# WLBF/flex-gpu-scheduler

Hardware: AMD Instinct MI355X
Metric: pods/sec sched throughput + p99 PodGroup gang-admit latency, 1/2/4/8-GPU groups (higher is better)
Workload: dtype int64

## Files before the change

csrc/api/types.cc:

```cpp
#include "api/types.h"

#include <algorithm>
#include <charconv>
#include <chrono>
#include <cstdio>
#include <cstdlib>
#include <limits>
#include <mutex>
#include <unordered_set>

#include "api/storage.h"

namespace xsched {

namespace {
int64_t days_from_civil(int64_t y, unsigned m, unsigned d) {
  y -= m <= 2;
  const int64_t era = (y >= 0 ? y : y - 399) / 400;
  const unsigned yoe = static_cast<unsigned>(y - era * 400);
  const unsigned doy = (153 * (m + (m > 2 ? -3 : 9)) + 2) / 5 + d - 1;
  const unsigned doe = yoe * 365 + yoe / 4 - yoe / 100 + doy;
  return era * 146097 + static_cast<int64_t>(doe) - 719468;
}
void civil_from_days(int64_t z, int64_t* y, unsigned* m, unsigned* d) {
// ... 342 lines not shown
    gpu.kind = GpuAssignment::Kind::Partition;
  } else if (limits.has(mid)) {
    gpu.kind = GpuAssignment::Kind::Memory;
    gpu.memory = limits.get(mid);
  } else {
    return;
  }
  gpu.gpus = std::move(gpus);
  gpu.partitions = std::move(parts);
}

const std::string& IStr::intern(std::string_view v) {
  static const std::string* kCommon[] = {new std::string(kDefaultSchedulerName), new std::string("PreemptLowerPriority"),
                                         new std::string("")};
  for (const std::string* c : kCommon)
    if (*c == v) return *c;
  static std::mutex mu;
  static auto* table = new std::unordered_set<std::string>();
  std::lock_guard<std::mutex> g(mu);
  return *table->emplace(v).first;
}

uint64_t pg_key_of(std::string_view full) {
  uint64_t h = 1469598103934665603ULL;
  for (unsigned char c : full) {
    h ^= c;
    h *= 1099511628211ULL;
  }
  return h ? h : 1;
}

std::shared_ptr<Pod> Pod::from_json(const Json& obj, const GpuNames& gn) {
  auto p = std::make_shared<Pod>();
  p->meta = ObjectMeta::from_json(obj);
  const Json& spec = obj["spec"];
  const Json& status = obj["status"];
  p->spec_hash = json_hash(spec, 1469598103934665603ULL, "nodeName");
  if (spec["nodeName"].as_string().empty()) {
    const Json& md = obj["metadata"];
    uint64_t h = json_hash(md["namespace"], p->spec_hash);
    p->template_hash = json_hash(md["annotations"], h);
  }
  if (spec["schedulerName"].is_string()) p->scheduler_name = spec["schedulerName"].as_string();
  p->node_name = spec["nodeName"].as_string();
  p->priority_class_name = spec["priorityClassName"].as_string();
  p->priority = as_i32(spec["priority"]);
  if (spec["preemptionPolicy"].is_string()) p->preemption_policy = spec["preemptionPolicy"].as_string();
  {
    std::vector<Container> cs, ics;
    for (const auto& c : spec["containers"].items()) cs.push_back(parse_container(c));
    for (const auto& c : spec["initContainers"].items()) ics.push_back(parse_container(c));
    p->containers = std::move(cs);
    p->init_containers = std::move(ics);
  }
  p->volumes = parse_pod_volumes(spec, p->meta.name);
  auto res = std::make_shared<PodRes>();
  res->overhead = Res::from_json(spec["overhead"]);
  p->node_selector = strmap_from_json(spec["nodeSelector"]);
  if (const Json* na = spec.path({"affinity", "nodeAffinity"})) {
    if (const Json* req = na->get("requiredDuringSchedulingIgnoredDuringExecution")) {
      p->has_required_node_affinity = true;
      for (const auto& t : (*req)["nodeSelectorTerms"].items()) p->required_node_terms.push_back(parse_term(t));
    }
    for (const auto& t : (*na)["preferredDuringSchedulingIgnoredDuringExecution"].items()) {
      PreferredSchedulingTerm pt;
      pt.weight = as_i32(t["weight"]);
      pt.pref = parse_term(t["preference"]);
      p->preferred_node_terms.push_back(std::move(pt));
    }
  }
  if (const Json* pa = spec.path({"affinity", "podAffinity"}))
    parse_pod_affinity(*pa, &p->pod_affinity_required, &p->pod_affinity_preferred);
  if (const Json* paa = spec.path({"affinity", "podAntiAffinity"}))
    parse_pod_affinity(*paa, &p->pod_anti_affinity_required, &p->pod_anti_affinity_preferred);
  for (const auto& c : spec["topologySpreadConstraints"].items()) {
    TopologySpreadConstraint tc;
    tc.max_skew = as_i32(c["maxSkew"], 1);
    tc.topology_key = c["topologyKey"].as_string();
    tc.hard = c["whenUnsatisfiable"].str_or("DoNotSchedule") != "ScheduleAnyway";
    tc.selector = LabelSelector::from_json(c.get("labelSelector"));
    p->spread_constraints.push_back(std::move(tc));
  }
  for (const auto& t : spec["tolerations"].items()) {
    Toleration tol;
    tol.key = t["key"].as_string();
    tol.op = t["operator"].str_or("Equal");
    tol.value = t["value"].as_string();
    tol.effect = t["effect"].as_string();
    if (t["tolerationSeconds"].is_number()) tol.toleration_seconds = t["tolerationSeconds"].as_int();
    p->tolerations.push_back(std::move(tol));
  }
  if (status["phase"].is_string()) p->phase = status["phase"].as_string();
  p->nominated_node_name = status["nominatedNodeName"].as_string();
  if (status["startTime"].is_string()) p->start_time = parse_rfc3339(status["startTime"].as_string());
  for (const auto& c : status["conditions"].items())
    if (c["type"].as_string() == "PodScheduled" && c["status"].as_string() == "True")
      p->scheduled_at = parse_rfc3339(c["lastTransitionTime"].as_string());

  Res sum;
  for (const auto& c : p->containers) {
    add_saturating(sum, c.requests);
    add_saturating(res->limit_sum, c.limits);
    Res nz;
    nz.set(kCPU, c.requests.has(kCPU) && c.requests.get(kCPU) != 0 ? c.requests.get(kCPU) : kDefaultMilliCPU);
    nz.set(kMemory, c.requests.has(kMemory) && c.requests.get(kMemory) != 0 ? c.requests.get(kMemory) : kDefaultMemory);
    add_saturating(res->nonzero_request, nz);
    for (const auto& port : c.ports)
      if (port.host_port > 0) p->host_ports.push_back(port);
  }
  if (p->containers.empty()) {
    res->nonzero_request.set(kCPU, 0);
    res->nonzero_request.set(kMemory, 0);
  }
  for (const auto& c : p->init_containers) {
    sum.set_max(c.requests);
    Res nz;
    nz.set(kCPU, c.requests.has(kCPU) && c.requests.get(kCPU) != 0 ? c.requests.get(kCPU) : kDefaultMilliCPU);
    nz.set(kMemory, c.requests.has(kMemory) && c.requests.get(kMemory) != 0 ? c.requests.get(kMemory) : kDefaultMemory);
    res->nonzero_request.set_max(nz);
  }
  add_saturating(sum, res->overhead);
  add_saturating(res->nonzero_request, res->overhead);
  res->request = sum;
  p->res = std::move(res);
  p->qos = compute_qos(*p);
  if (const std::string* pg = p->meta.label(kPodGroupLabel)) {
    p->pod_group = *pg;
    p->pg_key = pg_key_of(p->pg_full_name());
  }
  p->gpu_demand = compute_gpu_demand(*p, gn);
  p->recompute_gpu_assignment(gn);
  return p;
}

int partitions_for_mode(const std::string& mode) {
  std::string m;
  for (char c : mode) m.push_back(static_cast<char>(std::tolower(static_cast<unsigned char>(c))));
  if (m == "spx") return 1;
  if (m == "dpx") return 2;
  if (m == "qpx") return 4;
  if (m == "cpx") return 8;
  return 0;
}

bool node_selector_term_matches(const NodeSelectorTerm& t, const Node& n) {
  if (t.match_expressions.empty() && t.match_fields.empty()) return false;
  for (const auto& r : t.match_expressions)
    if (!match_requirement(r, n.meta.labels)) return false;
  for (const auto& r : t.match_fields) {
    if (r.key != "metadata.name") return false;
    StrMap f{{"metadata.name", n.name()}};
    if (!match_requirement(r, f)) return false;
  }
  return true;
}

bool pod_matches_node_selector_and_affinity(const Pod& p, const Node& n) {
  for (const auto& kv : p.node_selector) {
    const std::string* v = n.meta.label(kv.first);
    if (!v || *v != kv.second) return false;
  }
  if (!p.has_required_node_affinity) return true;
  for (const auto& t : p.required_node_terms)
    if (node_selector_term_matches(t, n)) return true;
  return false;
// ... 228 lines not shown
```

csrc/api/types.h:

```cpp
#pragma once

#include <atomic>
#include <cstdint>
#include <memory>
#include <optional>
#include <string>
#include <string_view>
#include <unordered_map>
#include <vector>

#include "api/resource.h"
#include "common/json.h"

namespace xsched {

inline constexpr const char* kPodGroupLabel = "pod-group.scheduling.sigs.k8s.io";
inline constexpr const char* kDefaultSchedulerName = "default-scheduler";

using MicroTime = int64_t;
MicroTime parse_rfc3339(const std::string& s);
std::string format_rfc3339(MicroTime t);
MicroTime wall_now_us();

using StrMap = std::vector<std::pair<std::string, std::string>>;
// ... 239 lines not shown
  };
  mutable ListedMark listed;
  struct HeapTag {
    uint8_t v = 0;
    HeapTag() = default;
    HeapTag(const HeapTag&) {}
    HeapTag& operator=(const HeapTag&) { return *this; }
  };
  mutable HeapTag heap_tag;

  std::shared_ptr<const PodRes> res = PodRes::empty();
  const Res& request() const { return res->request; }
  const Res& nonzero_request() const { return res->nonzero_request; }
  const Res& limit_sum() const { return res->limit_sum; }
  const Res& overhead() const { return res->overhead; }
  QoS qos = QoS::BestEffort;
  std::string pod_group;
  uint64_t pg_key = 0;
  std::shared_ptr<Gang> gang;
  std::vector<ContainerPort> host_ports;
  GpuAssignment gpu;
  GpuDemand gpu_demand;
  uint64_t template_hash = 0;
  uint64_t spec_hash = 0;

  const std::string& ns() const { return meta.ns; }
  const std::string& name() const { return meta.name; }
  const std::string& uid() const { return meta.uid; }
  std::string key() const { return meta.ns + "/" + meta.name; }
  bool terminating() const { return meta.deletion != 0; }
  std::string pg_full_name() const { return pod_group.empty() ? std::string() : meta.ns + "/" + pod_group; }

  static std::shared_ptr<Pod> from_json(const Json& obj, const GpuNames& gn = default_gpu_names());
  void recompute_gpu_assignment(const GpuNames& gn = default_gpu_names());
  void set_gpu_assignment(std::vector<int> gpus, std::vector<std::pair<int, int>> parts,
                          const GpuNames& gn = default_gpu_names());
};
using PodPtr = std::shared_ptr<Pod>;

uint64_t pg_key_of(std::string_view full_name);

struct Node {
  ObjectMeta meta;
  Res allocatable, capacity;
  bool unschedulable = false;
  std::vector<Taint> taints;
  std::vector<ContainerImage> images;
  std::unordered_map<std::string, int64_t> image_sizes;
  bool has_prefer_no_schedule = false;
  bool foreign_hostname = false;
  int gpu_count = 0;
  std::vector<int> gpu_partitions;
  std::vector<int> gpu_numa;
  std::vector<uint8_t> gpu_xcd_faults;
  int64_t gpu_memory_per_gpu = 0;
  const std::string& name() const { return meta.name; }
  static std::shared_ptr<Node> from_json(const Json& obj, const GpuNames& gn = default_gpu_names());
};
using NodePtr = std::shared_ptr<Node>;

bool node_selector_term_matches(const NodeSelectorTerm& t, const Node& n);
bool pod_matches_node_selector_and_affinity(const Pod& p, const Node& n);

struct PodGroup {
  ObjectMeta meta;
  int32_t min_member = 0;
// ... 96 lines not shown
```

csrc/python/bindings.cc:

```cpp
#include <pybind11/functional.h>
#include <pybind11/pybind11.h>
#include <pybind11/stl.h>

#include <atomic>
#include <map>
#include <set>

#include "api/types.h"
#include "common/alloc.h"
#include "common/json.h"
#include "common/quantity.h"
#include "rest/kube.h"
#include "scheduler/openloop.h"
#include "common/log.h"
#include "apiserver/apiserver.h"
#include "scheduler/scheduler.h"
#include "store/store.h"
#include "telemetry/amdsmi_sampler.h"
#include "tools/sampler.h"

namespace py = pybind11;
using namespace xsched;

namespace {
// ... 82 lines not shown
};

py::dict pod_struct_summary(const Pod& pod);

py::dict pod_summary(const Json& obj) { return pod_struct_summary(*Pod::from_json(obj)); }

py::dict pod_struct_summary(const Pod& pod) {
  const Pod* p = &pod;
  py::dict d;
  d["key"] = p->key();
  d["request"] = to_py(p->request().to_json());
  d["nonzero_request"] = to_py(p->nonzero_request().to_json());
  d["limits"] = to_py(p->limit_sum().to_json());
  const char* q[] = {"BestEffort", "Burstable", "Guaranteed"};
  d["qos"] = q[static_cast<int>(p->qos)];
  d["pod_group"] = p->pod_group;
  d["priority"] = p->priority;
  d["gpus"] = p->gpu.gpus;
  py::list parts;
  for (auto [g, pp] : p->gpu.partitions) parts.append(py::make_tuple(g, pp));
  d["partitions"] = parts;
  d["node_name"] = p->node_name;
  d["uid"] = p->uid();
  d["resource_version"] = p->meta.resource_version;
  d["labels"] = p->meta.labels.get();
  d["annotations"] = p->meta.annotations.get();
  d["phase"] = p->phase;
  d["scheduled_at"] = static_cast<int64_t>(p->scheduled_at);
  d["start_time"] = static_cast<int64_t>(p->start_time);
  d["template_hash"] = p->template_hash;
  d["spec_hash"] = p->spec_hash;
  d["scheduler_name"] = p->scheduler_name.str();
  d["host_ports"] = static_cast<int>(p->host_ports.size());
  return d;
}

py::dict node_info_dict(const NodeInfo& ni) {
  py::dict d;
  d["name"] = ni.name();
  d["pods"] = ni.num_pods();
  d["requested"] = to_py(ni.requested.to_json());
  d["allocatable"] = to_py(ni.allocatable.to_json());
  py::dict g;
  g["gpu_count"] = ni.gpu.gpu_count;
  g["mem_per_gpu"] = ni.gpu.mem_per_gpu;
  g["partitions"] = ni.gpu.parts;
  g["monopoly"] = ni.gpu.monopoly;
  py::list slots, fenced;
  for (int gi = 0; gi < ni.gpu.gpu_count; ++gi) {
    py::list ps, fs;
    for (int s = ni.gpu.offset[gi]; s < ni.gpu.offset[gi + 1]; ++s) {
      const auto& sl = ni.gpu.slots[s];
      ps.append(py::make_tuple(sl.exclusive, sl.used_mem, sl.mem_pods));
      fs.append(sl.fenced);
    }
    slots.append(ps);
    fenced.append(fs);
  }
  g["slots"] = slots;
  g["fenced"] = fenced;
  g["free_gpus"] = ni.gpu.free_gpus();
  g["free_xcds"] = ni.gpu.free_xcds();
  g["free_memory"] = ni.gpu.free_memory();
  d["gpu"] = g;
  return d;
}
// ... 47 lines not shown
  m.def("canonical_quantity", [](const std::string& s) { return Quantity::parse(s).str(); });
  m.def("quantity_cmp", [](const std::string& a, const std::string& b) {
    return Quantity::parse(a).cmp(Quantity::parse(b));
  });
  m.def("resource_list_op", [](const std::map<std::string, std::string>& a,
                               const std::map<std::string, std::string>& b, const std::string& op) {
    std::map<std::string, std::string> out;
    std::set<std::string> keys;
    for (const auto& kv : a) keys.insert(kv.first);
    for (const auto& kv : b) keys.insert(kv.first);
    for (const auto& k : keys) {
      auto ia = a.find(k), ib = b.find(k);
      bool ha = ia != a.end(), hb = ib != b.end();
      Quantity qa = ha ? Quantity::parse(ia->second) : Quantity();
      Quantity qb = hb ? Quantity::parse(ib->second) : Quantity();
      if (op == "max") {
        out[k] = (!ha || (hb && qb.cmp(qa) > 0) ? qb : qa).str();
        continue;
      }
      if (op != "add" && op != "sub") throw std::invalid_argument("op must be add, sub or max");
      if (qa.is_zero() && !ha) {
        qa = Quantity::from_int(0, qb.format());
      }
      if (op == "add") {
        qa.add(qb);
      } else {
        qa.sub(qb);
      }
      out[k] = qa.str();
    }
    return out;
  });
  m.def("pod_summary", [](py::handle obj) { return pod_summary(json_arg(obj)); });
  m.def("plugin_names", [] {
    register_builtin_plugins();
    return Registry::global().names();
  });
  m.def("json_roundtrip", [](const std::string& s) { return Json::parse(s).dump(); });
  m.def("json_parse", [](py::handle text) { return to_py(Json::parse(text_arg(text))); });
  m.def("json_dump", [](py::handle obj) { return py::bytes(from_py(obj).dump()); });
  m.def("json_hash", [](py::handle v) {
    bool text = py::isinstance<py::str>(v) || py::isinstance<py::bytes>(v);
    return json_hash(text ? Json::parse(text_arg(v)) : from_py(v));
  });
  m.def("json_parse_array_stream", [](py::handle text) {
    py::list out;
    Json::parse_array_stream(text_arg(text), [&](Json&& j) { out.append(to_py(j)); });
    return out;
  });
  m.def("amdsmi_status", [] {
    auto& smi = telemetry::AmdSmi::get();
    py::gil_scoped_release nogil;
    bool ok = smi.available();
    py::gil_scoped_acquire gil;
    return py::make_tuple(ok, smi.error());
  });
  m.def("amdsmi_sample", [] {
    std::vector<telemetry::GpuSample> v;
    {
      py::gil_scoped_release nogil;
      v = telemetry::AmdSmi::get().sample();
    }
    py::list out;
    for (const auto& s : v) {
      py::dict d;
      d["index"] = s.index;
// ... 303 lines not shown
      .def(py::init([](std::shared_ptr<ObjectStore> store, py::handle config, std::shared_ptr<FakeClock> clock,
                       std::shared_ptr<ApiClient> client) {
             Json cfg = json_arg(config);
             std::shared_ptr<Clock> c = clock;
             Scheduler* s;
             {
               py::gil_scoped_release r;
               s = new Scheduler(store, cfg, c, client);
             }
             return std::shared_ptr<Scheduler>(s, release_scheduler);
           }),
           py::arg("store"), py::arg("config"), py::arg("clock") = nullptr, py::arg("client") = nullptr)
      .def("start", &Scheduler::start, py::call_guard<py::gil_scoped_release>())
      .def("stop", &Scheduler::stop, py::call_guard<py::gil_scoped_release>())
      .def("sync_informers", &Scheduler::sync_informers, py::arg("timeout_ms") = 0,
           py::call_guard<py::gil_scoped_release>())
      .def("schedule_one", &Scheduler::schedule_one, py::arg("timeout_ms") = 0,
           py::call_guard<py::gil_scoped_release>())
      .def("wait_idle", &Scheduler::wait_idle, py::arg("timeout_ms") = 10000, py::call_guard<py::gil_scoped_release>())
      .def("stats",
           [](Scheduler& s) {
             auto st = s.stats();
             py::dict d;
             d["attempts"] = st.attempts;
             d["scheduled"] = st.scheduled;
             d["unschedulable"] = st.unschedulable;
             d["errors"] = st.errors;
             d["bound"] = st.bound;
             d["bind_failures"] = st.bind_failures;
             d["preemption_attempts"] = st.preemption_attempts;
             d["eq_filter_hits"] = st.eq_filter_hits;
             d["eq_filter_misses"] = st.eq_filter_misses;
             d["scan_memo_served"] = st.scan_memo_served;
             d["scan_memo_mismatches"] = st.scan_memo_mismatches;
             d["inflight_bindings"] = s.inflight_bindings();
             d["bind_threads"] = s.bind_threads();
             return d;
           })
      .def(
          "gang_records",
          [](Scheduler& s, bool clear) {
            py::list out;
            for (const auto& r : s.gang_records(clear)) {
              py::dict d;
              d["pod_group"] = r.pg;
              d["size"] = r.size;
              d["first_enqueue_us"] = r.first_enqueue_us;
              d["admit_us"] = r.admit_us;
              d["bound_us"] = r.bound_us;
              d["nodes"] = static_cast<int>(r.nodes.size());
              d["hostable"] = r.hostable;
              out.append(d);
            }
            return out;
          },
          py::arg("clear") = false)
      .def(
          "gang_denials",
          [](Scheduler& s, bool clear) {
            uint64_t total = 0;
            auto v = s.gang_denials(clear, &total);
            py::list out;
            for (const auto& d : v) {
              py::dict e;
              e["pod_group"] = d.pg;
              e["why"] = d.why;
// ... 174 lines not shown
```

csrc/scheduler/scheduler.cc:

```cpp
#include "scheduler/scheduler.h"

#include "common/log.h"

#include <algorithm>
#include <chrono>
#include <stdexcept>
#include <thread>

namespace xsched {

SchedulerOptions SchedulerOptions::from_json(const Json& j) {
  SchedulerOptions o;
  o.parallelism = static_cast<int>(j["parallelism"].as_int(o.parallelism));
  o.bind_workers = static_cast<int>(j["bindWorkers"].as_int(o.bind_workers));
  o.parallel_inline_below = static_cast<int>(j["parallelInlineBelow"].as_int(o.parallel_inline_below));
  o.percentage_of_nodes_to_score = static_cast<int>(j["percentageOfNodesToScore"].as_int(0));
  if (j["podInitialBackoffSeconds"].is_number())
    o.pod_initial_backoff_us = static_cast<int64_t>(j["podInitialBackoffSeconds"].as_double() * 1e6);
  if (j["podMaxBackoffSeconds"].is_number())
    o.pod_max_backoff_us = static_cast<int64_t>(j["podMaxBackoffSeconds"].as_double() * 1e6);
  if (j["assumedPodTTLSeconds"].is_number())
    o.assumed_pod_ttl_us = static_cast<int64_t>(j["assumedPodTTLSeconds"].as_double() * 1e6);
  o.metrics_sample_rate = j["metricsSampleRate"].as_double(o.metrics_sample_rate);
  o.status_updates = j["statusUpdates"].as_bool(o.status_updates);
  o.events = j["events"].as_bool(o.events);
  o.equivalence_cache = j["equivalenceCache"].as_bool(o.equivalence_cache);
  auto env_on = [](const char* var) {
    const char* v = std::getenv(var);
    return !v || std::string(v) != "0";
  };
  o.gang_window = j["gangWindow"].as_bool(env_on("XSCHED_GANG_WINDOW"));
  o.scan_memo = j["scanMemo"].as_bool(env_on("XSCHED_SCAN_MEMO"));
  o.scan_memo_verify = j["scanMemoVerify"].as_bool(false);
  o.trace = j["trace"].as_bool(false);
  o.seed = static_cast<uint64_t>(j["seed"].as_int(0));
  o.dump_on_fit_error = j["dumpOnFitError"].str_or("");
  o.gang_denial_census = j["gangDenialCensus"].as_bool(false);
  return o;
}

namespace {
const std::vector<std::string> kBaseKinds = {"pods", "nodes", "podgroups", "elasticquotas", "noderesourcetopologies",
                                             "poddisruptionbudgets", "priorityclasses"};
}

Scheduler::Scheduler(std::shared_ptr<ObjectStore> store, const Json& config, std::shared_ptr<Clock> clock,
                     std::shared_ptr<ApiClient> client)
    : store_(std::move(store)), clock_(clock ? std::move(clock) : std::make_shared<RealClock>()) {
  register_builtin_plugins();
  opts_ = SchedulerOptions::from_json(config["options"]);
  rng_.seed(opts_.seed ? opts_.seed : static_cast<uint64_t>(clock_->now_us()));
  tracer_.enable(opts_.trace);
  timers_ = std::make_unique<TimerService>(clock_);
  parallelizer_ = std::make_unique<Parallelizer>(opts_.parallelism, opts_.parallel_inline_below);
  if (const char* v = std::getenv("XSCHED_INFORMER_WINDOW")) informer_window_ = std::max<size_t>(1, std::atoll(v));
  if (const char* v = std::getenv("XSCHED_PARSE_POOL"); v && std::string(v) == "1")
    parse_pool_ = std::make_unique<Parallelizer>(4, 32, "xs-parse");
  metrics_ = std::make_unique<Metrics>();
  cache_ = std::make_unique<SchedulerCache>(clock_, opts_.assumed_pod_ttl_us);
  informers_ = std::make_unique<Informers>();
  nominator_ = std::make_unique<Nominator>();
  if (client) {
    client_ = std::move(client);
  } else {
    auto sc = std::make_shared<StoreClient>(store_);
    sc->events_enabled = opts_.events;
    client_ = std::move(sc);
  }

  for (const auto& ej : config["extenders"].items())
    extenders_.push_back(std::make_shared<Extender>(ExtenderConfig::from_json(ej)));
  const auto& profiles = config["profiles"].items();
  if (profiles.empty()) throw std::runtime_error("scheduler config has no profiles");
  for (const auto& pj : profiles) {
    const Json* args = pj["pluginConfig"].get("FlexGPU");
    if (!args) continue;
    auto gn = GpuNames::from_args(*args);
    if (!gpu_names_) gpu_names_ = gn;
    else if (!(*gn == *gpu_names_))
      throw std::runtime_error("FlexGPU resource names differ between profiles of one scheduler (" +
                               gpu_names_->describe() + " vs " + gn->describe() + ")");
  }
  if (!gpu_names_) gpu_names_ = std::make_shared<GpuNames>();
  cache_->set_gpu_names(gpu_names_.get());
  for (const auto& pj : profiles) {
    ProfileConfig pc = ProfileConfig::from_json(pj);
    if (pc.percentage_of_nodes_to_score == 0) pc.percentage_of_nodes_to_score = opts_.percentage_of_nodes_to_score;
    if (by_name_.count(pc.scheduler_name)) throw std::runtime_error("duplicate profile " + pc.scheduler_name);
    waiting_.push_back(std::make_unique<WaitingPods>(timers_.get()));
    Handle h;
// ... 114 lines not shown
  queue_->close();
  if (informer_thread_.joinable()) informer_thread_.join();
  if (sched_thread_.joinable()) sched_thread_.join();
  for (uint64_t id : timer_ids_) timers_->cancel(id);
  timer_ids_.clear();
  for (auto& w : waiting_) w->reject_all("scheduler stopped");
  if (binder_) binder_->stop();
  if (status_writer_) status_writer_->stop();
  if (was_running)
    for (auto& fw : frameworks_) fw->stop();
  timers_->stop();
}

Framework* Scheduler::framework_for(const std::string& scheduler_name) {
  auto it = by_name_.find(scheduler_name);
  return it == by_name_.end() ? nullptr : it->second;
}

bool Scheduler::responsible_for(const Pod& p) const { return by_name_.count(p.scheduler_name) > 0; }

Scheduler::Stats Scheduler::stats() const {
  Stats st;
  auto rd = [](const std::atomic<uint64_t>& a) { return a.load(std::memory_order_relaxed); };
  st.attempts = rd(cnt_.attempts);
  st.scheduled = rd(cnt_.scheduled);
  st.unschedulable = rd(cnt_.unschedulable);
  st.errors = rd(cnt_.errors);
  st.bound = rd(cnt_.bound);
  st.bind_failures = rd(cnt_.bind_failures);
  st.preemption_attempts = rd(cnt_.preemption_attempts);
  st.eq_filter_hits = rd(cnt_.eq_filter_hits);
  st.eq_filter_misses = rd(cnt_.eq_filter_misses);
  st.scan_memo_served = rd(cnt_.scan_memo_served);
  st.scan_memo_mismatches = rd(cnt_.scan_memo_mismatches);
  return st;
}

double Scheduler::loop_age_seconds() const {
  int64_t t = loop_tick_us_.load(std::memory_order_relaxed);
  if (!t || !running_.load()) return 0.0;
  return static_cast<double>(RealClock().now_us() - t) / 1e6;
}

void Scheduler::scheduling_loop() {
  RealClock rc;
  while (running_.load()) {
    loop_tick_us_.store(rc.now_us(), std::memory_order_relaxed);
    int64_t cycle = 0;
    auto qpi = queue_->pop(100, &cycle);
    if (!qpi) continue;
    std::lock_guard<std::mutex> g(sched_mu_);
    in_cycle_.fetch_add(1);
    schedule_cycle(qpi, cycle);
    in_cycle_.fetch_sub(1);
  }
}

bool Scheduler::schedule_one(int timeout_ms) {
  int64_t cycle = 0;
  auto qpi = queue_->pop(timeout_ms, &cycle);
  if (!qpi) return false;
  std::lock_guard<std::mutex> g(sched_mu_);
  in_cycle_.fetch_add(1);
  schedule_cycle(qpi, cycle);
  in_cycle_.fetch_sub(1);
  return true;
// ... 38 lines not shown
```

csrc/scheduler/scheduler.h:

```cpp
#pragma once

#include "common/adaptive_mutex.h"

#include <atomic>
#include <condition_variable>
#include <deque>
#include <functional>
#include <map>
#include <memory>
#include <mutex>
#include <random>
#include <string>
#include <thread>
#include <unordered_map>
#include <vector>

#include "common/clock.h"
#include "common/parallel.h"
#include "framework/framework.h"
#include "scheduler/cache.h"
#include "scheduler/executor.h"
#include "scheduler/extender.h"
#include "scheduler/gang_placement.h"
#include "scheduler/informers.h"
#include "scheduler/metrics.h"
#include "scheduler/queue.h"
#include "scheduler/trace.h"
#include "store/store.h"

namespace xsched {

class StoreClient : public ApiClient {
 public:
  explicit StoreClient(std::shared_ptr<ObjectStore> s) : store_(std::move(s)) {}
  void bind(const Pod& pod, const std::string& node, const Json& annotations) override;
  void delete_pod(const Pod& pod) override;
  void patch(const std::string& kind, const std::string& ns, const std::string& name, const Json& patch) override;
  void record_event(const std::string& kind, const std::string& ns, const std::string& name, const std::string& type,
                    const std::string& reason, const std::string& msg) override;
  bool events_enabled = false;

 private:
  std::shared_ptr<ObjectStore> store_;
  static constexpr int64_t kAggregateUs = 600LL * 1000000;
  struct Recent {
    std::string ns, name;
    int64_t count = 0, last_us = 0;
  };
  std::mutex events_mu_;
// ... 36 lines not shown
class Scheduler {
 public:
  Scheduler(std::shared_ptr<ObjectStore> store, const Json& config, std::shared_ptr<Clock> clock = nullptr,
            std::shared_ptr<ApiClient> client = nullptr);
  ~Scheduler();

  void start();
  void stop();
  size_t sync_informers(int timeout_ms = 0);
  bool schedule_one(int timeout_ms = 0);
  bool wait_idle(int timeout_ms);
  Json explain(const Json& pod);
  Json check_cache() const;
  Json dump_cache() const;
  double score_benchmark(const Json& pod, int iterations, Json* out = nullptr);
  Json plugin_call(const std::string& plugin, const std::string& point, const Json& args);

  SchedulingQueue& queue() { return *queue_; }
  SchedulerCache& cache() { return *cache_; }
  Informers& informers() { return *informers_; }
  Metrics& metrics() { return *metrics_; }
  Tracer& tracer() { return tracer_; }
  TimerService& timers() { return *timers_; }
  Framework* framework_for(const std::string& scheduler_name);
  const std::vector<std::unique_ptr<Framework>>& frameworks() const { return frameworks_; }
  std::shared_ptr<Clock> clock() const { return clock_; }
  std::shared_ptr<ObjectStore> store() const { return store_; }

  struct Stats {
    uint64_t attempts = 0, scheduled = 0, unschedulable = 0, errors = 0, bound = 0, bind_failures = 0;
    uint64_t preemption_attempts = 0;
    uint64_t eq_filter_hits = 0, eq_filter_misses = 0;
    uint64_t scan_memo_served = 0, scan_memo_mismatches = 0;
  };
  Stats stats() const;
  bool wait_bound(uint64_t target, int64_t timeout_us) const;
  bool wait_cache_empty(int64_t timeout_us) const;
  std::vector<GangRecord> gang_records(bool clear = false);
  std::vector<GangDenial> gang_denials(bool clear = false, uint64_t* total = nullptr);
  uint64_t gang_parks(bool clear = false);
  size_t inflight_bindings() const { return inflight_.load(); }
  size_t bind_threads() const { return binder_ ? binder_->threads() : 0; }
  size_t permit_waiting() const {
    size_t n = 0;
    for (const auto& w : waiting_) n += w->size();
    return n;
  }
  size_t bind_backlog() const { return binder_ ? binder_->pending() : 0; }
  double loop_age_seconds() const;

 private:
  struct Diagnosis {
    NodeStatusMap node_to_status;
    std::set<std::string> unschedulable_plugins;
  };

  void scheduling_loop();
  bool responsible_for(const Pod& p) const;

  std::shared_ptr<ObjectStore> store_;
  std::shared_ptr<Clock> clock_;
  SchedulerOptions opts_;
  std::unique_ptr<TimerService> timers_;
  std::unique_ptr<Parallelizer> parallelizer_;
  std::unique_ptr<Parallelizer> parse_pool_;
  ParallelSite parse_site_;
  std::unique_ptr<Metrics> metrics_;
  std::unique_ptr<SchedulerCache> cache_;
  std::unique_ptr<Informers> informers_;
  std::unique_ptr<Nominator> nominator_;
  std::unique_ptr<SchedulingQueue> queue_;
  std::shared_ptr<ApiClient> client_;
  ExtenderList extenders_;
  const ObjectLookup store_lookup_ = [this](const std::string& kind, const std::string& ns, const std::string& name) {
    return store_->get(kind, ns, name);
  };
  std::shared_ptr<const GpuNames> gpu_names_;
  std::vector<std::unique_ptr<WaitingPods>> waiting_;
  std::vector<std::unique_ptr<GangPlacement>> gang_placements_;
  std::vector<std::unique_ptr<Framework>> frameworks_;
  std::unordered_map<std::string, Framework*> by_name_;
  std::unique_ptr<Executor> binder_;
  std::unique_ptr<Executor> status_writer_;
  Snapshot snapshot_;
  Tracer tracer_;
  WatcherPtr watcher_;
  std::vector<std::string> plugin_kinds_;

  std::thread informer_thread_, sched_thread_;
  std::atomic<bool> running_{false};
  std::mutex sched_mu_;
  std::atomic<int> inflight_{0};
  std::atomic<int> in_cycle_{0};
  std::atomic<int64_t> loop_tick_us_{0};
  std::mt19937_64 rng_;
  std::vector<uint64_t> timer_ids_;
  struct Counters {
    std::atomic<uint64_t> attempts{0}, scheduled{0}, unschedulable{0}, errors{0}, bound{0}, bind_failures{0};
    std::atomic<uint64_t> preemption_attempts{0}, eq_filter_hits{0}, eq_filter_misses{0};
    std::atomic<uint64_t> scan_memo_served{0}, scan_memo_mismatches{0};
  } cnt_;
  std::atomic<uint64_t> bound_total_{0};

  void informer_loop();
  void handle_event(const WatchEvent& ev);
  void handle_pod_event(const WatchEvent& ev);
  void handle_pod_deletes(const WatchEvent* evs, size_t n);
  PodPtr deleted_pod(const WatchEvent& ev);
  void forget_unassigned_pod(const Pod& p);
  void capacity_freed();
  void report_informer_error(const WatchEvent& ev, const char* what);
  void handle_parsed_pod_event(const WatchEvent& ev, const PodPtr& np, PodPtr old);
  PodPtr bound_copy_of_assumed(const WatchEvent& ev);
  PodPtr status_copy_of_listed(const WatchEvent& ev);
  PodPtr copy_for_modified(const WatchEvent& ev) {
    PodPtr p = bound_copy_of_assumed(ev);
    return p ? p : status_copy_of_listed(ev);
  }
  void apply_pod_update(const WatchEvent& ev, const PodPtr& np, PodPtr old);
  void handle_node_event(const WatchEvent& ev);
  static constexpr size_t kInformerWindow = 64;
  size_t informer_window_ = kInformerWindow;

  void note_gang_enqueue(const Pod& p, int64_t t);
  void note_gang_event(const Pod& p, bool bound);
  void note_gang_planned(const Pod& p, bool hostable);
  void note_gang_denied(const Pod& p, const char* why);
  template <typename F>
  void with_gang_record(const Pod& p, bool open, GangRecord* done, F&& fn);
  mutable std::mutex stats_mu_;
  std::deque<GangRecord> gang_done_;
  std::unordered_map<int, Histogram*> gang_hist_;
  uint64_t gang_hist_epoch_ = ~0ULL;
// ... 114 lines not shown
```

csrc/scheduler/scheduler_events.cc:

```cpp
#include "scheduler/scheduler.h"

#include "common/log.h"
#include "common/reaper.h"

#include <algorithm>

namespace xsched {

namespace {
std::string resource_for_kind(const std::string& kind) {
  if (kind == "pods") return "Pod";
  if (kind == "nodes") return "Node";
  if (kind == "podgroups") return "PodGroup";
  if (kind == "elasticquotas") return "ElasticQuota";
  if (kind == "noderesourcetopologies") return "NodeResourceTopology";
  if (kind == "poddisruptionbudgets") return "PodDisruptionBudget";
  if (kind == "priorityclasses") return "PriorityClass";
  if (kind == "persistentvolumes") return "PersistentVolume";
  if (kind == "persistentvolumeclaims") return "PersistentVolumeClaim";
  if (kind == "storageclasses") return "StorageClass";
  if (kind == "csinodes") return "CSINode";
  return kind;
}
uint32_t action_for(EventType t) {
  switch (t) {
    case EventType::Added: return kAdd;
    case EventType::Deleted: return kDelete;
    default: return kUpdate;
  }
}
int64_t resource_version_of(const Json& obj) {
  const Json& rv = obj["metadata"]["resourceVersion"];
  return rv.is_string() ? std::atoll(rv.as_string().c_str()) : rv.as_int();
}
void refresh_version_and_status(Pod& np, const Json& obj) {
  np.meta.resource_version = resource_version_of(obj);
  const Json& status = obj["status"];
  np.phase = status["phase"].is_string() ? status["phase"].as_string() : std::string("Pending");
  np.nominated_node_name = status["nominatedNodeName"].as_string();
  np.start_time = status["startTime"].is_string() ? parse_rfc3339(status["startTime"].as_string()) : 0;
  np.scheduled_at = 0;
  for (const auto& c : status["conditions"].items())
    if (c["type"].as_string() == "PodScheduled" && c["status"].as_string() == "True")
      np.scheduled_at = parse_rfc3339(c["lastTransitionTime"].as_string());
}
}

void Scheduler::informer_loop() {
  while (running_.load()) {
    auto evs = watcher_->next(50, 8192);
    if (evs.empty()) continue;
    int64_t batch_start = tracer_.enabled() ? clock_->now_us() : 0;
    std::vector<PodPtr> parsed(evs.size());
    std::vector<PodPtr> prev(evs.size());
    std::vector<size_t> to_parse;
    auto group_of = [](const WatchEvent& ev) -> const std::string& {
      return (*ev.obj)["metadata"]["labels"][kPodGroupLabel].as_string();
    };
    size_t lo = 0;
    while (lo < evs.size()) {
      size_t hi = lo;
      while (hi < evs.size()) {
        const auto& ev = evs[hi];
        if (hi - lo >= informer_window_) {
          const auto& pe = evs[hi - 1];
          bool same_group = ev.kind == "pods" && pe.kind == "pods" && ev.type == EventType::Added &&
                            pe.type == EventType::Added && !group_of(ev).empty() && group_of(ev) == group_of(pe);
          if (!same_group) break;
        }
        ++hi;
        if (ev.kind != "pods" || ev.type == EventType::Deleted) continue;
        try {
          if (ev.type == EventType::Modified) parsed[hi - 1] = copy_for_modified(ev);
        } catch (const std::exception&) {
          continue;
        }
        if (!parsed[hi - 1]) to_parse.push_back(hi - 1);
      }
      if (!to_parse.empty()) {
        auto parse_one = [&](int k) {
          const size_t i = to_parse[static_cast<size_t>(k)];
          try {
            parsed[i] = Pod::from_json(*evs[i].obj, *gpu_names_);
          } catch (const std::exception&) {
          }
        };
        if (parse_pool_) {
          parse_pool_->until(static_cast<int>(to_parse.size()), parse_one, nullptr, &parse_site_);
        } else {
          for (size_t k = 0; k < to_parse.size(); ++k) parse_one(static_cast<int>(k));
        }
        to_parse.clear();
      }
      informers_->upsert_pods(&parsed[lo], &prev[lo], hi - lo);
      for (size_t i = lo; i < hi;) {
        if (!parsed[i] && evs[i].type == EventType::Deleted && evs[i].kind == "pods") {
          size_t j = i + 1;
          while (j < hi && evs[j].type == EventType::Deleted && evs[j].kind == "pods") ++j;
          if (j - i > 1) {
            handle_pod_deletes(&evs[i], j - i);
            i = j;
            continue;
          }
        }
        if (parsed[i])
          handle_parsed_pod_event(evs[i], parsed[i], prev[i]);
        else
          handle_event(evs[i]);
        parsed[i].reset();
        prev[i].reset();
        ++i;
      }
      lo = hi;
    }
    if (tracer_.enabled() && batch_start)
      tracer_.record(TraceEvent{"informer_batch", std::to_string(evs.size()) + " events", "", batch_start,
                                clock_->now_us() - batch_start, 2});
  }
}

size_t Scheduler::sync_informers(int timeout_ms) {
  size_t n = 0;
  for (;;) {
    auto evs = watcher_->next(n == 0 ? timeout_ms : 0, 8192);
    if (evs.empty()) break;
// ... 282 lines not shown
```

flex_gpu_scheduler_amd/build_ext.py:

```python
from __future__ import annotations

import argparse
import concurrent.futures as cf
import os
import shutil
import subprocess
import sys
import sysconfig
from pathlib import Path

ROOT = Path(__file__).resolve().parent.parent
CSRC = ROOT / "csrc"
PKG = ROOT / "flex_gpu_scheduler_amd"
BUILD = ROOT / "build"
HIP_ARCH = os.environ.get("PYTORCH_ROCM_ARCH", "gfx950")
ROCM = Path(os.environ.get("ROCM_PATH", "/opt/rocm"))

CORE_DIRS = ["common", "api", "store", "framework", "scheduler", "plugins", "rest", "apiserver"]
LINK_LIBS = ["-lssl", "-lcrypto"]
CXXFLAGS = ["-std=c++20", "-O3", "-fPIC", "-Wall", "-Wno-unused-variable", "-Wno-unused-parameter",
            "-Wno-sign-compare", "-fvisibility=hidden", "-pthread",
            *os.environ.get("XSCHED_CXXFLAGS_EXTRA", "").split()]


# ... 254 lines not shown
    out = BUILD / ("xsched_gang_tests_tsan" if tsan else "xsched_gang_tests")
    newest = max(o.stat().st_mtime for o in objs)
    if out.exists() and out.stat().st_mtime >= newest:
        return out
    cmd = ["g++", *(["-fsanitize=thread"] if tsan else []), "-pthread", *[str(o) for o in objs], *LINK_LIBS,
           "-o", str(out)]
    r = subprocess.run(cmd, capture_output=True, text=True)
    if r.returncode != 0:
        raise RuntimeError(f"gang tests link failed:\n{r.stderr[-8000:]}")
    if verbose:
        print(f"[build_ext] built {out.relative_to(ROOT)}")
    return out


def build_assume_tests(verbose: bool = True, tsan: bool = False) -> Path:
    includes = [str(CSRC)]
    extra = ["-fsanitize=thread", "-g", "-O1", "-include", str(CSRC / "tools" / "tsan_compat.h")] if tsan else []
    objs = build_objects(core_sources() + [CSRC / "tests" / "assume_tests.cc"], BUILD / ("tsan" if tsan else "core"),
                         extra, includes)
    out = BUILD / ("xsched_assume_tests_tsan" if tsan else "xsched_assume_tests")
    newest = max(o.stat().st_mtime for o in objs)
    if out.exists() and out.stat().st_mtime >= newest:
        return out
    cmd = ["g++", *(["-fsanitize=thread"] if tsan else []), "-pthread", *[str(o) for o in objs], *LINK_LIBS,
           "-o", str(out)]
    r = subprocess.run(cmd, capture_output=True, text=True)
    if r.returncode != 0:
        raise RuntimeError(f"assume tests link failed:\n{r.stderr[-8000:]}")
    if verbose:
        print(f"[build_ext] built {out.relative_to(ROOT)}")
    return out


def build_wire_tests(verbose: bool = True, sanitize: bool = False) -> Path:
    flags = ["-fsanitize=address,undefined", "-fno-sanitize-recover=all", "-fno-omit-frame-pointer"] if sanitize else []
    srcs = [CSRC / "rest" / "wire.cc", CSRC / "tests" / "wire_tests.cc"]
    objs = build_objects(srcs, BUILD / ("wire_asan" if sanitize else "core"), [*flags, "-g", "-O1"] if sanitize else [],
                         [str(CSRC)])
    out = BUILD / ("xsched_wire_tests_asan" if sanitize else "xsched_wire_tests")
    newest = max(o.stat().st_mtime for o in objs)
    if out.exists() and out.stat().st_mtime >= newest:
        return out
    cmd = ["g++", *flags, "-pthread", *[str(o) for o in objs], *LINK_LIBS, "-o", str(out)]
    r = subprocess.run(cmd, capture_output=True, text=True)
    if r.returncode != 0:
        raise RuntimeError(f"wire tests link failed:\n{r.stderr[-8000:]}")
    if verbose:
        print(f"[build_ext] built {out.relative_to(ROOT)}")
    return out


def main(argv: list[str] | None = None) -> int:
    ap = argparse.ArgumentParser()
    ap.add_argument("--core", action="store_true")
    ap.add_argument("--hip", action="store_true")
    ap.add_argument("--tsan", action="store_true")
    ap.add_argument("--asan", action="store_true")
    ap.add_argument("--json-fuzz", action="store_true", help="JSON/pod-decode driver under ASan+UBSan (host only)")
    ap.add_argument("--patch-fuzz", action="store_true", help="JSON patch / selector driver under ASan+UBSan (host only)")
    ap.add_argument("--prof", action="store_true")
    ap.add_argument("--stress", action="store_true")
    ap.add_argument("--stress-g", action="store_true", help="stress driver with -g (sample_report --lines)")
    ap.add_argument("--stress-count", action="store_true",
                    help="stress driver with the counting operator new/delete (allocations per thread)")
    ap.add_argument("--stress-count-g", action="store_true", help="the same with line tables (call stacks)")
    ap.add_argument("--tests", action="store_true")
    ap.add_argument("--core-g", action="store_true", help="the extension with -g into dbg/ (sampling runs)")
    ap.add_argument("--gang-tests", action="store_true", help="native tests of the lister's gang entries")
    ap.add_argument("--gang-tests-tsan", action="store_true", help="the same under ThreadSanitizer (host only)")
    ap.add_argument("--assume-tests", action="store_true",
                    help="native tests of assume-with-placement, pop's cycle number and append_int")
    ap.add_argument("--assume-tests-tsan", action="store_true", help="the same under ThreadSanitizer (host only)")
    ap.add_argument("--wire-tests", action="store_true", help="native tests of the HTTP/1.1 wire layer")
    ap.add_argument("--wire-asan", action="store_true", help="the same under ASan+UBSan (host only)")
    a = ap.parse_args(argv)
    if a.wire_tests or a.wire_asan:
        build_wire_tests(sanitize=a.wire_asan)
        return 0
    if a.gang_tests or a.gang_tests_tsan:
        build_gang_tests(tsan=a.gang_tests_tsan)
        return 0
    if a.assume_tests or a.assume_tests_tsan:
        build_assume_tests(tsan=a.assume_tests_tsan)
        return 0
    if a.core_g:
        build_core_debuginfo()
        return 0
    if a.json_fuzz:
        build_json_fuzz()
        return 0
    if a.patch_fuzz:
        build_patch_fuzz()
        return 0
    if a.tests:
        build_tests()
        return 0
    if a.stress_count or a.stress_count_g:
        build_stress_count(debuginfo=a.stress_count_g)
        return 0
    if a.prof or a.stress or a.stress_g:
        build_prof(gprof=a.prof, debuginfo=a.stress_g)
        return 0
    everything = not (a.core or a.hip or a.tsan or a.asan)
    if a.core or everything:
        build_core()
    if a.hip or everything:
        build_hip()
    if a.tsan:
        build_tsan()
    if a.asan:
        build_asan()
    return 0


if __name__ == "__main__":
    sys.exit(main())
# ... 1 lines not shown
```

Baseline: 145,300.

## Memoize pod spec decoding across Added events with identical specs

Adds a direct-mapped memo keyed by spec hash that reuses a previously decoded Pod for Added events whose spec is identical, copying it and re-deriving only the per-object fields (metadata, status, pod group, GPU assignment). Pod::from_json is split so that the object-specific parts live in a new set_object_fields method. The informer loop also skips parsing Added/Modified events for pods deleted earlier in the same window. It is on by default unless the parse pool is enabled. The costs are a full spec hash plus a deep JSON equality compare per Added event and a Pod copy, and the memo risks reusing stale derived state if any field depends on metadata.

After: 138,700. 4.6% lower.

```diff
diff --git a/csrc/api/pod_memo.cc b/csrc/api/pod_memo.cc
--- /dev/null
+++ b/csrc/api/pod_memo.cc
@@ -0,0 +1,37 @@
+#include "api/pod_memo.h"
+
+#include <algorithm>
+
+namespace xsched {
+
+PodDecodeMemo::PodDecodeMemo(size_t slots) : slots_(std::max<size_t>(1, slots)) {}
+
+std::shared_ptr<Pod> PodDecodeMemo::decode(const JsonPtr& obj, const GpuNames& gn) {
+  const Json& spec = (*obj)["spec"];
+  if (!spec["nodeName"].as_string().empty() || !spec["volumes"].items().empty()) {
+    ++bypassed_;
+    return Pod::from_json(*obj, gn);
+  }
+  const uint64_t spec_hash = json_hash(spec, 1469598103934665603ULL, "nodeName");
+  Slot& slot = slots_[spec_hash % slots_.size()];
+  if (slot.decoded && slot.spec_hash == spec_hash && slot.gn == &gn && (*slot.source)["spec"] == spec) {
+    auto p = std::make_shared<Pod>(*slot.decoded);
+    p->set_object_fields(*obj, gn);
+    ++hits_;
+    return p;
+  }
+  auto p = Pod::from_json(*obj, gn);
+  auto kept = std::make_shared<Pod>(*p);
+  kept->meta = ObjectMeta{};
+  kept->gpu = GpuAssignment{};
+  kept->pod_group.clear();
+  kept->nominated_node_name.clear();
+  slot.spec_hash = spec_hash;
+  slot.source = obj;
+  slot.decoded = std::move(kept);
+  slot.gn = &gn;
+  ++misses_;
+  return p;
+}
+
+}
diff --git a/csrc/api/pod_memo.h b/csrc/api/pod_memo.h
--- /dev/null
+++ b/csrc/api/pod_memo.h
@@ -0,0 +1,33 @@
+#pragma once
+
+#include <cstddef>
+#include <cstdint>
+#include <memory>
+#include <vector>
+
+#include "api/types.h"
+#include "common/json.h"
+
+namespace xsched {
+
+class PodDecodeMemo {
+ public:
+  explicit PodDecodeMemo(size_t slots = 256);
+  std::shared_ptr<Pod> decode(const JsonPtr& obj, const GpuNames& gn);
+
+  uint64_t hits() const { return hits_; }
+  uint64_t misses() const { return misses_; }
+  uint64_t bypassed() const { return bypassed_; }
+
+ private:
+  struct Slot {
+    uint64_t spec_hash = 0;
+    JsonPtr source;
+    std::shared_ptr<const Pod> decoded;
+    const GpuNames* gn = nullptr;
+  };
+  std::vector<Slot> slots_;
+  uint64_t hits_ = 0, misses_ = 0, bypassed_ = 0;
+};
+
+}
diff --git a/csrc/api/types.cc b/csrc/api/types.cc
--- a/csrc/api/types.cc
+++ b/csrc/api/types.cc
@@ -398,15 +398,8 @@
 
 std::shared_ptr<Pod> Pod::from_json(const Json& obj, const GpuNames& gn) {
   auto p = std::make_shared<Pod>();
-  p->meta = ObjectMeta::from_json(obj);
   const Json& spec = obj["spec"];
-  const Json& status = obj["status"];
   p->spec_hash = json_hash(spec, 1469598103934665603ULL, "nodeName");
-  if (spec["nodeName"].as_string().empty()) {
-    const Json& md = obj["metadata"];
-    uint64_t h = json_hash(md["namespace"], p->spec_hash);
-    p->template_hash = json_hash(md["annotations"], h);
-  }
   if (spec["schedulerName"].is_string()) p->scheduler_name = spec["schedulerName"].as_string();
   p->node_name = spec["nodeName"].as_string();
   p->priority_class_name = spec["priorityClassName"].as_string();
@@ -419,7 +412,7 @@
     p->containers = std::move(cs);
     p->init_containers = std::move(ics);
   }
-  p->volumes = parse_pod_volumes(spec, p->meta.name);
+  p->volumes = parse_pod_volumes(spec, obj["metadata"]["name"].as_string());
   auto res = std::make_shared<PodRes>();
   res->overhead = Res::from_json(spec["overhead"]);
   p->node_selector = strmap_from_json(spec["nodeSelector"]);
@@ -456,12 +449,6 @@
     if (t["tolerationSeconds"].is_number()) tol.toleration_seconds = t["tolerationSeconds"].as_int();
     p->tolerations.push_back(std::move(tol));
   }
-  if (status["phase"].is_string()) p->phase = status["phase"].as_string();
-  p->nominated_node_name = status["nominatedNodeName"].as_string();
-  if (status["startTime"].is_string()) p->start_time = parse_rfc3339(status["startTime"].as_string());
-  for (const auto& c : status["conditions"].items())
-    if (c["type"].as_string() == "PodScheduled" && c["status"].as_string() == "True")
-      p->scheduled_at = parse_rfc3339(c["lastTransitionTime"].as_string());
 
   Res sum;
   for (const auto& c : p->containers) {
@@ -490,13 +477,34 @@
   res->request = sum;
   p->res = std::move(res);
   p->qos = compute_qos(*p);
-  if (const std::string* pg = p->meta.label(kPodGroupLabel)) {
-    p->pod_group = *pg;
-    p->pg_key = pg_key_of(p->pg_full_name());
-  }
   p->gpu_demand = compute_gpu_demand(*p, gn);
-  p->recompute_gpu_assignment(gn);
+  p->set_object_fields(obj, gn);
   return p;
+}
+
+void Pod::set_object_fields(const Json& obj, const GpuNames& gn) {
+  meta = ObjectMeta::from_json(obj);
+  template_hash = 0;
+  if (node_name.empty()) {
+    const Json& md = obj["metadata"];
+    uint64_t h = json_hash(md["namespace"], spec_hash);
+    template_hash = json_hash(md["annotations"], h);
+  }
+  const Json& status = obj["status"];
+  phase = status["phase"].is_string() ? status["phase"].as_string() : std::string("Pending");
+  nominated_node_name = status["nominatedNodeName"].as_string();
+  start_time = status["startTime"].is_string() ? parse_rfc3339(status["startTime"].as_string()) : 0;
+  scheduled_at = 0;
+  for (const auto& c : status["conditions"].items())
+    if (c["type"].as_string() == "PodScheduled" && c["status"].as_string() == "True")
+      scheduled_at = parse_rfc3339(c["lastTransitionTime"].as_string());
+  pod_group.clear();
+  pg_key = 0;
+  if (const std::string* pg = meta.label(kPodGroupLabel)) {
+    pod_group = *pg;
+    pg_key = pg_key_of(pg_full_name());
+  }
+  recompute_gpu_assignment(gn);
 }
 
 int partitions_for_mode(const std::string& mode) {
diff --git a/csrc/api/types.h b/csrc/api/types.h
--- a/csrc/api/types.h
+++ b/csrc/api/types.h
@@ -295,6 +295,7 @@
   std::string pg_full_name() const { return pod_group.empty() ? std::string() : meta.ns + "/" + pod_group; }
 
   static std::shared_ptr<Pod> from_json(const Json& obj, const GpuNames& gn = default_gpu_names());
+  void set_object_fields(const Json& obj, const GpuNames& gn = default_gpu_names());
   void recompute_gpu_assignment(const GpuNames& gn = default_gpu_names());
   void set_gpu_assignment(std::vector<int> gpus, std::vector<std::pair<int, int>> parts,
                           const GpuNames& gn = default_gpu_names());
diff --git a/csrc/python/bindings.cc b/csrc/python/bindings.cc
--- a/csrc/python/bindings.cc
+++ b/csrc/python/bindings.cc
@@ -138,6 +138,11 @@
   d["spec_hash"] = p->spec_hash;
   d["scheduler_name"] = p->scheduler_name.str();
   d["host_ports"] = static_cast<int>(p->host_ports.size());
+  d["nominated_node_name"] = p->nominated_node_name;
+  py::list claims;
+  for (const auto& v : p->volumes)
+    if (v.kind == PodVolume::Kind::PVC || v.kind == PodVolume::Kind::Ephemeral) claims.append(v.claim);
+  d["volume_claims"] = claims;
   return d;
 }
 
@@ -251,6 +256,28 @@
     return out;
   });
   m.def("pod_summary", [](py::handle obj) { return pod_summary(json_arg(obj)); });
+  m.def(
+      "pod_summaries_memo",
+      [](py::iterable texts, size_t slots, bool raise_errors) {
+        PodDecodeMemo memo(slots);
+        py::list out;
+        for (py::handle t : texts) {
+          auto doc = std::make_shared<const Json>(json_arg(t));
+          try {
+            out.append(pod_struct_summary(*memo.decode(doc, default_gpu_names())));
+          } catch (const std::invalid_argument& e) {
+            if (raise_errors) throw;
+            out.append(py::module_::import("builtins").attr("ValueError")(e.what()));
+          }
+        }
+        py::dict d;
+        d["summaries"] = out;
+        d["hits"] = memo.hits();
+        d["misses"] = memo.misses();
+        d["bypassed"] = memo.bypassed();
+        return d;
+      },
+      py::arg("texts"), py::arg("slots") = 256, py::arg("raise_errors") = true);
   m.def("plugin_names", [] {
     register_builtin_plugins();
     return Registry::global().names();
@@ -620,6 +647,9 @@
              d["eq_filter_hits"] = st.eq_filter_hits;
              d["eq_filter_misses"] = st.eq_filter_misses;
              d["scan_memo_served"] = st.scan_memo_served;
+             d["decode_memo_hits"] = st.decode_memo_hits;
+             d["decode_memo_misses"] = st.decode_memo_misses;
+             d["decode_memo_bypassed"] = st.decode_memo_bypassed;
              d["scan_memo_mismatches"] = st.scan_memo_mismatches;
              d["inflight_bindings"] = s.inflight_bindings();
              d["bind_threads"] = s.bind_threads();
diff --git a/csrc/scheduler/scheduler.cc b/csrc/scheduler/scheduler.cc
--- a/csrc/scheduler/scheduler.cc
+++ b/csrc/scheduler/scheduler.cc
@@ -56,6 +56,8 @@
   if (const char* v = std::getenv("XSCHED_INFORMER_WINDOW")) informer_window_ = std::max<size_t>(1, std::atoll(v));
   if (const char* v = std::getenv("XSCHED_PARSE_POOL"); v && std::string(v) == "1")
     parse_pool_ = std::make_unique<Parallelizer>(4, 32, "xs-parse");
+  if (const char* v = std::getenv("XSCHED_DECODE_MEMO"); !v || std::string(v) != "0")
+    decode_memo_ = std::make_unique<PodDecodeMemo>();
   metrics_ = std::make_unique<Metrics>();
   cache_ = std::make_unique<SchedulerCache>(clock_, opts_.assumed_pod_ttl_us);
   informers_ = std::make_unique<Informers>();
@@ -236,6 +238,9 @@
   st.eq_filter_hits = rd(cnt_.eq_filter_hits);
   st.eq_filter_misses = rd(cnt_.eq_filter_misses);
   st.scan_memo_served = rd(cnt_.scan_memo_served);
+  st.decode_memo_hits = rd(cnt_.decode_memo_hits);
+  st.decode_memo_misses = rd(cnt_.decode_memo_misses);
+  st.decode_memo_bypassed = rd(cnt_.decode_memo_bypassed);
   st.scan_memo_mismatches = rd(cnt_.scan_memo_mismatches);
   return st;
 }
diff --git a/csrc/scheduler/scheduler.h b/csrc/scheduler/scheduler.h
--- a/csrc/scheduler/scheduler.h
+++ b/csrc/scheduler/scheduler.h
@@ -15,6 +15,7 @@
 #include <unordered_map>
 #include <vector>
 
+#include "api/pod_memo.h"
 #include "common/clock.h"
 #include "common/parallel.h"
 #include "framework/framework.h"
@@ -117,6 +118,7 @@
     uint64_t preemption_attempts = 0;
     uint64_t eq_filter_hits = 0, eq_filter_misses = 0;
     uint64_t scan_memo_served = 0, scan_memo_mismatches = 0;
+    uint64_t decode_memo_hits = 0, decode_memo_misses = 0, decode_memo_bypassed = 0;
   };
   Stats stats() const;
   bool wait_bound(uint64_t target, int64_t timeout_us) const;
@@ -150,6 +152,7 @@
   std::unique_ptr<Parallelizer> parallelizer_;
   std::unique_ptr<Parallelizer> parse_pool_;
   ParallelSite parse_site_;
+  std::unique_ptr<PodDecodeMemo> decode_memo_;
   std::unique_ptr<Metrics> metrics_;
   std::unique_ptr<SchedulerCache> cache_;
   std::unique_ptr<Informers> informers_;
@@ -184,6 +187,7 @@
     std::atomic<uint64_t> attempts{0}, scheduled{0}, unschedulable{0}, errors{0}, bound{0}, bind_failures{0};
     std::atomic<uint64_t> preemption_attempts{0}, eq_filter_hits{0}, eq_filter_misses{0};
     std::atomic<uint64_t> scan_memo_served{0}, scan_memo_mismatches{0};
+    std::atomic<uint64_t> decode_memo_hits{0}, decode_memo_misses{0}, decode_memo_bypassed{0};
   } cnt_;
   std::atomic<uint64_t> bound_total_{0};
 
diff --git a/csrc/scheduler/scheduler_events.cc b/csrc/scheduler/scheduler_events.cc
--- a/csrc/scheduler/scheduler_events.cc
+++ b/csrc/scheduler/scheduler_events.cc
@@ -47,6 +47,7 @@
 }
 
 void Scheduler::informer_loop() {
+  PodDecodeMemo* const memo = parse_pool_ ? nullptr : decode_memo_.get();
   while (running_.load()) {
     auto evs = watcher_->next(50, 8192);
     if (evs.empty()) continue;
@@ -54,12 +55,14 @@
     std::vector<PodPtr> parsed(evs.size());
     std::vector<PodPtr> prev(evs.size());
     std::vector<size_t> to_parse;
+    std::vector<const Json*> deleted;
     auto group_of = [](const WatchEvent& ev) -> const std::string& {
       return (*ev.obj)["metadata"]["labels"][kPodGroupLabel].as_string();
     };
     size_t lo = 0;
     while (lo < evs.size()) {
       size_t hi = lo;
+      deleted.clear();
       while (hi < evs.size()) {
         const auto& ev = evs[hi];
         if (hi - lo >= informer_window_) {
@@ -69,7 +72,19 @@
           if (!same_group) break;
         }
         ++hi;
-        if (ev.kind != "pods" || ev.type == EventType::Deleted) continue;
+        if (ev.kind != "pods") continue;
+        if (ev.type == EventType::Deleted) {
+          deleted.push_back(&(*ev.obj)["metadata"]);
+          continue;
+        }
+        if (!deleted.empty()) {
+          const Json& md = (*ev.obj)["metadata"];
+          const std::string &ns = md["namespace"].as_string(), &name = md["name"].as_string();
+          bool recreated = false;
+          for (const Json* d : deleted)
+            if ((*d)["name"].as_string() == name && (*d)["namespace"].as_string() == ns) recreated = true;
+          if (recreated) continue;
+        }
         try {
           if (ev.type == EventType::Modified) parsed[hi - 1] = copy_for_modified(ev);
         } catch (const std::exception&) {
@@ -81,7 +96,8 @@
         auto parse_one = [&](int k) {
           const size_t i = to_parse[static_cast<size_t>(k)];
           try {
-            parsed[i] = Pod::from_json(*evs[i].obj, *gpu_names_);
+            parsed[i] = memo && evs[i].type == EventType::Added ? memo->decode(evs[i].obj, *gpu_names_)
+                                                                 : Pod::from_json(*evs[i].obj, *gpu_names_);
           } catch (const std::exception&) {
           }
         };
@@ -91,6 +107,11 @@
           for (size_t k = 0; k < to_parse.size(); ++k) parse_one(static_cast<int>(k));
         }
         to_parse.clear();
+        if (memo) {
+          cnt_.decode_memo_hits.store(memo->hits(), std::memory_order_relaxed);
+          cnt_.decode_memo_misses.store(memo->misses(), std::memory_order_relaxed);
+          cnt_.decode_memo_bypassed.store(memo->bypassed(), std::memory_order_relaxed);
+        }
       }
       informers_->upsert_pods(&parsed[lo], &prev[lo], hi - lo);
       for (size_t i = lo; i < hi;) {
diff --git a/flex_gpu_scheduler_amd/build_ext.py b/flex_gpu_scheduler_amd/build_ext.py
--- a/flex_gpu_scheduler_amd/build_ext.py
+++ b/flex_gpu_scheduler_amd/build_ext.py
@@ -310,6 +310,25 @@
     return out
 
 
+def build_decode_tests(verbose: bool = True, tsan: bool = False) -> Path:
+    includes = [str(CSRC)]
+    extra = ["-fsanitize=thread", "-g", "-O1", "-include", str(CSRC / "tools" / "tsan_compat.h")] if tsan else []
+    objs = build_objects(core_sources() + [CSRC / "tests" / "decode_tests.cc"], BUILD / ("tsan" if tsan else "core"),
+                         extra, includes)
+    out = BUILD / ("xsched_decode_tests_tsan" if tsan else "xsched_decode_tests")
+    newest = max(o.stat().st_mtime for o in objs)
+    if out.exists() and out.stat().st_mtime >= newest:
+        return out
+    cmd = ["g++", *(["-fsanitize=thread"] if tsan else []), "-pthread", *[str(o) for o in objs], *LINK_LIBS,
+           "-o", str(out)]
+    r = subprocess.run(cmd, capture_output=True, text=True)
+    if r.returncode != 0:
+        raise RuntimeError(f"decode tests link failed:\n{r.stderr[-8000:]}")
+    if verbose:
+        print(f"[build_ext] built {out.relative_to(ROOT)}")
+    return out
+
+
 def build_wire_tests(verbose: bool = True, sanitize: bool = False) -> Path:
     flags = ["-fsanitize=address,undefined", "-fno-sanitize-recover=all", "-fno-omit-frame-pointer"] if sanitize else []
     srcs = [CSRC / "rest" / "wire.cc", CSRC / "tests" / "wire_tests.cc"]
@@ -349,6 +368,9 @@
     ap.add_argument("--assume-tests", action="store_true",
                     help="native tests of assume-with-placement, pop's cycle number and append_int")
     ap.add_argument("--assume-tests-tsan", action="store_true", help="the same under ThreadSanitizer (host only)")
+    ap.add_argument("--decode-tests", action="store_true",
+                    help="native tests of the pod decode memo")
+    ap.add_argument("--decode-tests-tsan", action="store_true", help="the same under ThreadSanitizer (host only)")
     ap.add_argument("--wire-tests", action="store_true", help="native tests of the HTTP/1.1 wire layer")
     ap.add_argument("--wire-asan", action="store_true", help="the same under ASan+UBSan (host only)")
     a = ap.parse_args(argv)
@@ -360,6 +382,9 @@
         return 0
     if a.assume_tests or a.assume_tests_tsan:
         build_assume_tests(tsan=a.assume_tests_tsan)
+        return 0
+    if a.decode_tests or a.decode_tests_tsan:
+        build_decode_tests(tsan=a.decode_tests_tsan)
         return 0
     if a.core_g:
         build_core_debuginfo()
```
